# lliutianc/MPVAE-1

Measured on AMD Instinct MI355X. Metric: probit MC label-samples/sec (B×n_sample×L) at 1/2/4/8 GPU; ELBO rel-err, higher is better.
Workload: dtype f32; 1 GPU; c4: compute_loss fwd+bwd, B=512, L=1024, z=1024, n_sample=4096 (4096/GPU), philox noise on device; global_batch=512, n_sample=4096, label_dim=1024, z_dim=1024, parallelism=n_sample-sharded x1, gemm=f16x3

## Files before the change

mpvae-1_amd/csrc/mpv_common.h:

```cpp
#pragma once

#include <hip/hip_runtime.h>
#include <stdint.h>

#include "mpvae_hip.h"

#define MPV_DEV __device__ __forceinline__

namespace mpv {

constexpr float kEps1 = 1e-6f;
constexpr float kC1 = 1.0f - kEps1;
constexpr float kC0 = kEps1 * 0.5f;
constexpr float kInvSqrt2 = 0.70710678118654752440f;
constexpr float kInvSqrt2Pi = 0.39894228040143267794f;
constexpr float kKlEps = 1e-6f;
constexpr float kKlWeight = 1.1f;

typedef float f32x4 __attribute__((ext_vector_type(4)));

MPV_DEV float fast_log(float x) { return __builtin_amdgcn_logf(x) * 0.6931471805599453f; }
MPV_DEV float fast_rcp(float x) { return __builtin_amdgcn_rcpf(x); }

typedef float f32x2 __attribute__((ext_vector_type(2)));
// ... 238 lines not shown
      "v_fma_mixlo_f16 %1, %2, %3, -%0 op_sel_hi:[0,0,1]\n\t"
      "v_fma_mixhi_f16 %1, %2, %4, -%0 op_sel:[0,0,1] op_sel_hi:[0,0,1]"
      : "=&v"(h), "=&v"(l)
      : "s"(s), "v"(x0), "v"(x1), "v"(nz));
  hi = h;
  lo = l;
}

MPV_DEV float add_f32(float a, float b) {
  float r;
  asm("v_add_f32 %0, %1, %2" : "=v"(r) : "v"(a), "v"(b));
  return r;
}

MPV_DEV float pow2_scale(float maxabs) {
  if (!(maxabs > 0.0f) || !isfinite(maxabs)) return 1.0f;
  int e;
  frexpf(maxabs, &e);
  return ldexpf(1.0f, 14 - e);
}

MPV_DEV void bstat_combine_row(const float* __restrict__ g, int64_t R, int64_t B, int64_t b,
                               float (&v)[6]) {
#pragma unroll
  for (int br = 0; br < 2; ++br) {
    const int mi = 2 * br, zi = 2 * br + 1;
    float M = -INFINITY;
    for (int64_t r = 0; r < R; ++r) M = fmaxf(M, g[(r * 6 + mi) * B + b]);
    float Z = 0.0f;
    for (int64_t r = 0; r < R; ++r) Z += g[(r * 6 + zi) * B + b] * expf(g[(r * 6 + mi) * B + b] - M);
    v[mi] = M;
    v[zi] = Z;
  }
  for (int k = 4; k < 6; ++k) {
    float acc = 0.0f;
    for (int64_t r = 0; r < R; ++r) acc += g[(r * 6 + k) * B + b];
    v[k] = acc;
  }
}

MPV_DEV float wave_pow2_scale(const float* __restrict__ bound, int n) {
  float m = 0.0f;
  for (int i = threadIdx.x & 63; i < n; i += 64) m = fmaxf(m, bound[i]);
  return pow2_scale(wave_max(m));
}

MPV_DEV f16x8 as_f16x8(s16x8 v) { return __builtin_bit_cast(f16x8, v); }

constexpr int kLoOff = 32;
__host__ __device__ inline int64_t chunked_index(int64_t r, int64_t ld, int64_t c) {
  return r * ld + ((c >> 5) << 6) + (c & 31);
}

MPV_DEV void barrier_raw() {
  asm volatile("" ::: "memory");
  __builtin_amdgcn_s_barrier();
  asm volatile("" ::: "memory");
}

MPV_DEV void lds_barrier() {
  asm volatile("s_waitcnt lgkmcnt(0)" ::: "memory");
  barrier_raw();
}

template <int N>
MPV_DEV void wait_vmcnt() {
  asm volatile("s_waitcnt vmcnt(%0)" ::"n"(N) : "memory");
}

MPV_DEV uint32_t lds_addr(const void* p) {
  return (uint32_t)(uintptr_t)(const __attribute__((address_space(3))) void*)p;
}

MPV_DEV void lds_dma16(const void* saddr, uint32_t voff, uint32_t lds) {
  uint32_t keep;
  asm volatile(
      "s_mov_b32 %0, m0\n\ts_mov_b32 m0, %3\n\ts_nop 0\n\t"
      "global_load_lds_dwordx4 %1, %2\n\ts_mov_b32 m0, %0"
      : "=&s"(keep)
      : "v"(voff), "s"(saddr), "s"(lds)
      : "memory");
}

__host__ __device__ inline int64_t t_cols(int64_t L) { return (L + 3) & ~int64_t(3); }

MPV_DEV void wait_vmcnt_dyn(int n) {
#define MPV_VMC(k) \
  case k:          \
    wait_vmcnt<k>(); \
    break;
  switch (n) {
    MPV_VMC(0) MPV_VMC(1) MPV_VMC(2) MPV_VMC(3) MPV_VMC(4) MPV_VMC(5) MPV_VMC(6) MPV_VMC(7)
    MPV_VMC(8) MPV_VMC(9) MPV_VMC(10) MPV_VMC(11) MPV_VMC(12) MPV_VMC(13) MPV_VMC(14)
    MPV_VMC(15) MPV_VMC(16) MPV_VMC(17) MPV_VMC(18) MPV_VMC(19) MPV_VMC(20) MPV_VMC(21)
    MPV_VMC(22) MPV_VMC(23) MPV_VMC(24)
    default:
      wait_vmcnt<0>();
      break;
  }
#undef MPV_VMC
}

struct u32x4 { uint32_t x, y, z, w; };

MPV_DEV u32x4 philox4x32_10(u32x4 c, uint32_t k0, uint32_t k1) {
#pragma unroll
  for (int r = 0; r < 10; ++r) {
    const uint64_t p0 = (uint64_t)0xD2511F53u * c.x, p1 = (uint64_t)0xCD9E8D57u * c.z;
    const uint32_t lo0 = (uint32_t)p0, hi0 = (uint32_t)(p0 >> 32);
    const uint32_t lo1 = (uint32_t)p1, hi1 = (uint32_t)(p1 >> 32);
    c = u32x4{(uint32_t)__builtin_amdgcn_bitop3_b32(hi1, c.y, k0, 0x96), lo1,
              (uint32_t)__builtin_amdgcn_bitop3_b32(hi0, c.w, k1, 0x96), lo0};
    k0 += 0x9E3779B9u;
    k1 += 0xBB67AE85u;
  }
  return c;
}

MPV_DEV void box_muller(uint32_t we, uint32_t wo, float& n0, float& n1) {
  const float u = ((float)(we >> 8) + 0.5f) * 5.9604644775390625e-8f;
  const float v = (float)(wo >> 8) * 5.9604644775390625e-8f;
  const float r = __builtin_amdgcn_sqrtf(-1.3862943611198906f * __builtin_amdgcn_logf(u));
  n0 = r * __builtin_amdgcn_cosf(v);
  n1 = r * __builtin_amdgcn_sinf(v);
}

inline int num_cus() {
  static const int n = [] {
    int dev = 0, v = 0;
    if (hipGetDevice(&dev) != hipSuccess ||
        hipDeviceGetAttribute(&v, hipDeviceAttributeMultiprocessorCount, dev) != hipSuccess ||
        v <= 0)
      v = 256;
    return v;
  }();
  return n;
}

}
```

mpvae-1_amd/csrc/probit_bwd.hip:

```cpp
#include "abi_util.h"
#include "mpv_common.h"


namespace mpv {

int launch_sum_slabs(const float* in, int64_t nslab, int64_t n, void* out, int out_dtype,
                     hipStream_t s);
int launch_sum_slabs_pair(const float* in0, int64_t nslab0, int64_t n0, void* out0,
                          int out0_dtype, const float* in1, int64_t nslab1, int64_t n1,
                          void* out1, int out1_dtype, hipStream_t s);

constexpr float kBoundDl = 4.5f, kBoundPos = 0.4f, kBoundNeg = 60.0f, kBoundInd = 0.4f;

constexpr int kCoefThreads = 512;

__global__ __launch_bounds__(kCoefThreads) void bwd_coef_kernel(
    const float* __restrict__ y, const float* __restrict__ rowstat, const float* __restrict__ bstat,
    const float* __restrict__ gscal, const float* __restrict__ gI, const float* __restrict__ gIL,
    float* __restrict__ coef, float* __restrict__ gbound, int S, int B, int L, float S_total,
    float nll_coeff, float c_coeff, int live, mpv_kl_bwd_args kl, int kl_blocks) {
  __shared__ float red[48];
  if ((int)blockIdx.x >= B) {
    kl_bwd_range(kl, (int64_t)(blockIdx.x - B) * blockDim.x + threadIdx.x,
                 (int64_t)kl_blocks * blockDim.x);
    return;
  }
  const int b = blockIdx.x, tid = threadIdx.x;
  float np = 0.f, nn = 0.f, gi = 0.f;
  for (int l = tid; l < L; l += blockDim.x) {
    const int64_t o = (int64_t)b * L + l;
    const float v = y[o];
    np += (v == 1.0f) ? 1.0f : 0.0f;
    nn += (v == 0.0f) ? 1.0f : 0.0f;
    gi = fmaxf(gi, (gI ? fabsf(gI[o]) : 0.0f) + (gIL ? fabsf(gIL[o]) : 0.0f));
  }
  {
    const int lane = tid & 63, wid = tid >> 6, nw = (blockDim.x + 63) >> 6;
    np = wave_sum(np);
    nn = wave_sum(nn);
    gi = wave_max(gi);
    __syncthreads();
    if (lane == 0) red[wid] = np, red[16 + wid] = nn, red[32 + wid] = gi;
    __syncthreads();
    np = nn = 0.0f;
    gi = -INFINITY;
    for (int i = 0; i < nw; ++i) {
      np += red[i];
      nn += red[16 + i];
      gi = fmaxf(gi, red[32 + i]);
    }
  }
  const float nrm = np * nn;
  auto gs = [&](int k) { return (live & MPV_LIVE(k)) ? gscal[k] : 0.0f; };
  const float gt = gs(MPV_G_TOTAL);
  const float gn[2] = {gs(MPV_G_NLL) + nll_coeff * gt, gs(MPV_G_NLL_X) + nll_coeff * gt};
  const float gc[2] = {gs(MPV_G_C) + c_coeff * gt, gs(MPV_G_C_X) + c_coeff * gt};
  const bool clive[2] = {(live & (MPV_LIVE(MPV_G_TOTAL) | MPV_LIVE(MPV_G_C))) != 0,
                         (live & (MPV_LIVE(MPV_G_TOTAL) | MPV_LIVE(MPV_G_C_X))) != 0};
  const float inv_B = 1.0f / (float)B;
  float bound = kBoundInd * gi / S_total;
  float bmaxb[2];
#pragma unroll
  for (int br = 0; br < 2; ++br) {
    const float M = bstat[(2 * br) * B + b], Z = bstat[(2 * br + 1) * B + b];
    const bool dead = !(nrm > 0.0f) && clive[br];
    const float cs = gc[br] / (nrm * S_total * (float)B);
    float bmax = 0.0f;
    auto one = [&](float lp, float P, float N, float& ca, float& cp, float& cn) {
      float alpha = -gn[br] * (expf(lp - M) / Z) * inv_B;
      float bP = nrm > 0.0f ? cs * N : 0.0f;
      float bN = nrm > 0.0f ? cs * P : 0.0f;
      bmax = fmaxf(bmax, kBoundDl * fabsf(alpha) + kBoundPos * fabsf(bP) + kBoundNeg * fabsf(bN));
      if (dead) alpha = bP = bN = __builtin_nanf("");
      ca = alpha * kPhiK;
      cp = bP * kPhiK;
      cn = bN * kPhiK;
    };
    const float* rl = rowstat + ((int64_t)br * B + b) * S;
    const float* rp = rowstat + ((int64_t)(2 + 2 * br) * B + b) * S;
    const float* rn = rowstat + ((int64_t)(3 + 2 * br) * B + b) * S;
    float* ca = coef + ((int64_t)(3 * br + 0) * B + b) * S;
    float* cp = coef + ((int64_t)(3 * br + 1) * B + b) * S;
    float* cn = coef + ((int64_t)(3 * br + 2) * B + b) * S;
    if ((S & 3) == 0) {
      for (int s = 4 * tid; s < S; s += 4 * (int)blockDim.x) {
        const f32x4 lp = *reinterpret_cast<const f32x4*>(rl + s);
        const f32x4 P = *reinterpret_cast<const f32x4*>(rp + s);
        const f32x4 N = *reinterpret_cast<const f32x4*>(rn + s);
        float a[4], p[4], n[4];
#pragma unroll
        for (int j = 0; j < 4; ++j) one(lp[j], P[j], N[j], a[j], p[j], n[j]);
        *reinterpret_cast<f32x4*>(ca + s) = f32x4{a[0], a[1], a[2], a[3]};
        *reinterpret_cast<f32x4*>(cp + s) = f32x4{p[0], p[1], p[2], p[3]};
        *reinterpret_cast<f32x4*>(cn + s) = f32x4{n[0], n[1], n[2], n[3]};
      }
    } else {
      for (int s = tid; s < S; s += blockDim.x) one(rl[s], rp[s], rn[s], ca[s], cp[s], cn[s]);
    }
    bmaxb[br] = bmax;
  }
  block_reduce2<true>(bmaxb[0], bmaxb[1], red);
  bound += bmaxb[0];
  bound += bmaxb[1];
  if (tid == 0 && gbound) gbound[b] = bound;
}

struct ElemParams {
  const float* y;
  const float* fe;
  const float* fx;
  const float* gI;
  const float* gIL;
  const float* coef;
  float* T;
  uint16_t* g;
  const float* g_bound;
  int64_t gld;
  float* colpart;
  int S, B, L, Lc;
  int ldT;
  int TPR, RPI, rows_per_chunk;
  float inv_S;
};

struct ElemCol {
  f32x2 base[4];
  f32x2 gind[4];
  float y[4];
  bool soft[4];
  float qm[4];
  float sga[4];
  float wp[4], wn[4];
  bool pos[4];
  float kp, kn;
};

template <bool SOFT = true, bool NANCHK = true, bool SOFT_RCP = false>
MPV_DEV void d_elem2x4(const float (&t)[4], const ElemCol& c, f32x2 alpha, f32x2 rkp, f32x2 rkn,
                       f32x2 (&out)[4], const f32x2* rkq = nullptr, const f32x2* qc1 = nullptr) {
  f32x2 zq[4], w[4], ez[4];
#pragma unroll
  for (int q = 0; q < 4; ++q) zq[q] = pk_fma(splat2(t[q]), splat2(kZq), c.base[q]);
  probit_dw2xN_zq<4>(zq, w, ez, qc1);
#pragma unroll
  for (int q = 0; q < 4; ++q) {
    f32x2 E;
    {
#pragma clang fp contract(off)
      E = w[q] * kEh + splat2(kC0);
    }
    const f32x2 d = E + splat2(c.qm[q]);
    const f32x2 r = f32x2{fast_rcp(d.x), fast_rcp(d.y)};
    f32x2 dE;
    if (SOFT && c.soft[q]) {
      const f32x2 omE = splat2(1.0f) - E;
      const f32x2 dl = SOFT_RCP ? splat2(c.y[q]) * f32x2{fast_rcp(E.x), fast_rcp(E.y)} -
                                      splat2(1.0f - c.y[q]) * f32x2{fast_rcp(omE.x), fast_rcp(omE.y)}
                                : splat2(c.y[q]) / E - splat2(1.0f - c.y[q]) / omE;
      dE = pk_fma(alpha, dl, c.gind[q]);
    } else {
      dE = pk_fma(alpha, r, c.gind[q]);
    }
    const f32x2 rk = rkq   ? rkq[q]
                     : SOFT ? pk_fma(splat2(c.wn[q]), rkn, splat2(c.wp[q]) * rkp)
                            : (c.pos[q] ? rkp : rkn);
    const f32x2 a = w[q] * c.sga[q];
    dE = pk_fma(rk, f32x2{__builtin_amdgcn_exp2f(a.x), __builtin_amdgcn_exp2f(a.y)}, dE);
    out[q] = dE * ez[q];
  }
  if (NANCHK && (rkp.x != rkp.x || rkp.y != rkp.y)) {
#pragma unroll
    for (int q = 0; q < 4; ++q) {
      if (rkp.x != rkp.x) out[q].x = rkp.x;
      if (rkp.y != rkp.y) out[q].y = rkp.y;
    }
  }
}

MPV_DEV void elem_rank_coefs(const ElemCol& c, f32x2 bP, f32x2 bN, f32x2& rkp, f32x2& rkn) {
  rkp = splat2(c.kp) * -bP;
  rkn = splat2(c.kn) * bN;
}

struct ElemRow {
  f32x2 alpha, bP, bN;
  float t[4];
};

MPV_DEV void elem_row_load(ElemRow& r, const ElemParams& p, int b, int s, int c0,
                           const bool (&ok)[4]) {
  const int64_t cb = (int64_t)b * p.S + s;
  const int64_t BS = (int64_t)p.B * p.S;
  r.alpha = f32x2{p.coef[0 * BS + cb], p.coef[3 * BS + cb]};
  r.bP = f32x2{p.coef[1 * BS + cb], p.coef[4 * BS + cb]};
  r.bN = f32x2{p.coef[2 * BS + cb], p.coef[5 * BS + cb]};
  const float* row = p.T + cb * p.ldT;
  if (c0 < p.L) {
    const f32x4 v = __builtin_nontemporal_load(reinterpret_cast<const f32x4*>(row + c0));
    r.t[0] = v[0]; r.t[1] = v[1]; r.t[2] = v[2]; r.t[3] = v[3];
  } else {
#pragma unroll
    for (int q = 0; q < 4; ++q) r.t[q] = ok[q] ? row[c0 + q] : 0.0f;
  }
}

MPV_DEV void elem_col_setup(const ElemParams& p, int b, int c0, bool active, bool (&ok)[4],
                            ElemCol& ec) {
  const int L = p.L;
  ec.kp = exp2f((-5.0f * 1.4426950408889634f) * kC0);
  ec.kn = exp2f((5.0f * 1.4426950408889634f) * kC0);
#pragma unroll
  for (int q = 0; q < 4; ++q) {
    const int c = c0 + q;
    ok[q] = active && c < L;
    const int64_t o = (int64_t)b * L + (ok[q] ? c : 0);
    const float yv = ok[q] ? p.y[o] : 0.0f;
    const float fe = ok[q] ? p.fe[o] : 0.0f;
    const float fx = ok[q] ? p.fx[o] : 0.0f;
    const float gi = (ok[q] && p.gI) ? p.gI[o] * p.inv_S : 0.0f;
    const float gil = (ok[q] && p.gIL) ? p.gIL[o] * p.inv_S : 0.0f;
    ec.base[q] = f32x2{fe, fx} * kZq;
    ec.gind[q] = f32x2{gil, gi} * kPhiK;
    ec.y[q] = yv;
    ec.soft[q] = !(yv == 0.0f || yv == 1.0f);
    ec.qm[q] = yv == 0.0f ? -1.0f : 0.0f;
    const float sgx = (yv == 1.0f ? -5.0f : 5.0f) * 1.4426950408889634f;
    ec.sga[q] = sgx * kEh;
    ec.wp[q] = yv == 1.0f ? 1.0f : 0.0f;
    ec.wn[q] = yv == 0.0f ? 1.0f : 0.0f;
    ec.pos[q] = yv == 1.0f;
  }
}

constexpr int kElemLookahead = 1;
constexpr int kElemMinRows = 16;
template <bool PLANES>
__global__ __launch_bounds__(256, 3) void bwd_elem_kernel(ElemParams p) {
  constexpr int LA = kElemLookahead;
  __shared__ float cred[256 * 8];
  const int b = blockIdx.x, sc = blockIdx.y;
  const int tid = threadIdx.x;
  const int rsub = tid / p.TPR, cq = tid % p.TPR;
  const bool active = rsub < p.RPI;
  const int c0 = blockIdx.z * 1024 + cq * 4;
// ... 13 lines not shown
    for (int j = 0; j < LA; ++j)
      if (s0 + j * R < s_end) elem_row_load(buf[j], p, b, s0 + j * R, c0, ok);
    for (int s = s0; s < s_end; s += R) {
      if (s + LA * R < s_end) elem_row_load(buf[LA], p, b, s + LA * R, c0, ok);
      const ElemRow& cur = buf[0];
      const int64_t cb = (int64_t)b * S + s;
      float G[4];
      f32x2 g2[4];
      f32x2 rkp, rkn;
      elem_rank_coefs(ec, cur.bP, cur.bN, rkp, rkn);
      d_elem2x4(cur.t, ec, cur.alpha, rkp, rkn, g2);
#pragma unroll
      for (int q = 0; q < 4; ++q) {
        sg2[q] = sg2[q] + g2[q];
        G[q] = ok[q] ? g2[q].x + g2[q].y : 0.0f;
      }
      if (PLANES) {
        uint16_t h[4], l[4];
#pragma unroll
        for (int q = 0; q < 4; ++q) split_f16(G[q], gs, h[q], l[q]);
        const int64_t o = chunked_index(cb, p.gld, c0);
        const s16x4 hv{(short)h[0], (short)h[1], (short)h[2], (short)h[3]};
        const s16x4 lv{(short)l[0], (short)l[1], (short)l[2], (short)l[3]};
        __builtin_nontemporal_store(hv, reinterpret_cast<s16x4*>(p.g + o));
        __builtin_nontemporal_store(lv, reinterpret_cast<s16x4*>(p.g + o + kLoOff));
      } else {
        float* row = p.T + cb * p.ldT;
        if (c0 < L) {
          *reinterpret_cast<f32x4*>(row + c0) = f32x4{G[0], G[1], G[2], G[3]};
        } else {
#pragma unroll
          for (int q = 0; q < 4; ++q)
            if (ok[q]) row[c0 + q] = G[q];
        }
      }
#pragma unroll
      for (int j = 0; j < LA; ++j) buf[j] = buf[j + 1];
    }
  }
#pragma unroll
  for (int q = 0; q < 4; ++q) {
    cred[tid * 8 + q] = sg2[q].x;
    cred[tid * 8 + 4 + q] = sg2[q].y;
  }
  __syncthreads();
  for (int j = tid; j < p.TPR * 4; j += blockDim.x) {
    const int cqq = j >> 2, q = j & 3;
    const int c = blockIdx.z * 1024 + j;
    if (c < L) {
      float e = 0.f, x = 0.f;
      for (int r = 0; r < p.RPI; ++r) {
        e += cred[(r * p.TPR + cqq) * 8 + q];
        x += cred[(r * p.TPR + cqq) * 8 + 4 + q];
      }
      p.colpart[(((int64_t)sc * 2 + 0) * B + b) * L + c] = e;
      p.colpart[(((int64_t)sc * 2 + 1) * B + b) * L + c] = x;
    }
  }
}

constexpr int kElemRing = 8;
constexpr int kElemRingRows = 256;
constexpr int kElemRingMinRows = 128;
template <bool SOFT, bool MASK, bool NANCHK>
MPV_DEV void elem_ring_rows(const ElemParams& p, const ElemCol& ec, const bool (&ok)[4], bool live,
                            int b, int sb, int nrows, int c0, float gs, uint32_t voff,
                            float* myring, const float (*cf)[8], f32x2 (&sg2)[4]) {
  constexpr int NR = kElemRing;
  const int lane = threadIdx.x & 63;
  const int64_t rowb = (int64_t)b * p.S + sb;
  const char* tbase = reinterpret_cast<const char*>(p.T + rowb * p.ldT);
  const int64_t rstride = (int64_t)p.ldT * 4;
  auto issue = [&](int r) {
    lds_dma16(tbase + r * rstride, voff, lds_addr(myring + (r % NR) * 256));
  };
  const int pro = min(NR, nrows);
  for (int r = 0; r < pro; ++r) issue(r);
  uint32_t rsel[4];
#pragma unroll
  for (int q = 0; q < 4; ++q) rsel[q] = ec.pos[q] ? 0u : 16u;
  const uint32_t loffb = live ? 2u * (uint32_t)(((c0 >> 5) << 6) + (c0 & 31)) : 0u;
  f32x2 qc1 = splat2(kErfcxC1);
  asm volatile("" : "+v"(qc1));
  auto row = [&](int r) {
    const f32x4 tv = *reinterpret_cast<const f32x4*>(myring + (r % NR) * 256 + lane * 4);
    const float t[4] = {tv[0], tv[1], tv[2], tv[3]};
    f32x2 g2[4];
    const char* crow =
        reinterpret_cast<const char*>(&cf[0][0]) + __builtin_amdgcn_readfirstlane(r * 32);
    const f32x2 rkp = *reinterpret_cast<const f32x2*>(crow);
    const f32x2 rkn = *reinterpret_cast<const f32x2*>(crow + 16);
    if (SOFT) {
      const f32x2 alpha = *reinterpret_cast<const f32x2*>(crow + 8);
      d_elem2x4<SOFT, false, true>(t, ec, alpha, rkp, rkn, g2);
    } else {
      f32x2 rkq[4];
#pragma unroll
      for (int q = 0; q < 4; ++q) rkq[q] = *reinterpret_cast<const f32x2*>(crow + rsel[q]);
      const f32x2 alpha = *reinterpret_cast<const f32x2*>(crow + rsel[0] + 8);
      d_elem2x4<SOFT, false, true>(t, ec, alpha, rkp, rkn, g2, rkq, &qc1);
    }
    if (NANCHK && __builtin_amdgcn_readfirstlane((rkp.x != rkp.x || rkp.y != rkp.y) ? 1 : 0)) {
#pragma unroll
      for (int q = 0; q < 4; ++q) {
        if (rkp.x != rkp.x) g2[q].x = rkp.x;
        if (rkp.y != rkp.y) g2[q].y = rkp.y;
      }
    }
    float G[4];
#pragma unroll
    for (int q = 0; q < 4; ++q) {
      sg2[q] = sg2[q] + g2[q];
      G[q] = add_f32(g2[q].x, g2[q].y);
      if (MASK && !ok[q]) G[q] = 0.0f;
    }
    uint32_t hv[2], lv[2];
    split2_f16(G[0], G[1], gs, hv[0], lv[0]);
    split2_f16(G[2], G[3], gs, hv[1], lv[1]);
    const uint64_t ga = reinterpret_cast<uint64_t>(p.g + (rowb + r) * p.gld);
    const uint64_t grow =
        ((uint64_t)(uint32_t)__builtin_amdgcn_readfirstlane((uint32_t)(ga >> 32)) << 32) |
        (uint64_t)(uint32_t)__builtin_amdgcn_readfirstlane((uint32_t)ga);
    if (!MASK || live) {
      asm volatile("global_store_dwordx2 %0, %1, %2 nt\n\t"
                   "global_store_dwordx2 %0, %3, %2 offset:%4 nt"
                   :
                   : "v"(loffb), "v"(u32x2{hv[0], hv[1]}), "s"(grow), "v"(u32x2{lv[0], lv[1]}),
                     "i"(2 * kLoOff));
    }
    if (r + NR < nrows) issue(r + NR);
  };
  int r = 0;
  if (!SOFT && !MASK && !NANCHK) {
    for (; r < min(NR - 1, nrows); ++r) {
      wait_vmcnt_dyn(min(NR - 1, nrows - 1 - r) + 2 * r);
      row(r);
    }
    for (; r <= nrows - NR; ++r) {
      wait_vmcnt<3 * (NR - 1)>();
      row(r);
    }
  }
  for (; r < nrows; ++r) {
    wait_vmcnt_dyn(min(NR - 1, nrows - 1 - r) + 2 * min(r, NR - 1));
    row(r);
  }
}

__global__ __launch_bounds__(256, 3) void bwd_elem_ring_kernel(ElemParams p) {
  constexpr int NR = kElemRing, CR = kElemRingRows;
  __shared__ __attribute__((aligned(16))) float ring[4][NR][256];
  __shared__ __attribute__((aligned(16))) float cf[CR][8];
  const int b = blockIdx.x, sc = blockIdx.y, tid = threadIdx.x;
  const int wid = __builtin_amdgcn_readfirstlane(tid >> 6);
  const int c0 = blockIdx.z * 1024 + tid * 4;
  const int S = p.S, B = p.B, L = p.L;
  const float gs = wave_pow2_scale(p.g_bound, B);
  bool ok[4];
  ElemCol ec;
  elem_col_setup(p, b, c0, true, ok, ec);
  bool my_soft = false;
#pragma unroll
  for (int q = 0; q < 4; ++q) my_soft |= ok[q] && ec.soft[q];
  const bool soft_any = __syncthreads_or(my_soft) != 0;
  const bool wave_live = (int)(blockIdx.z * 1024 + wid * 256) < p.Lc;
  const bool wave_full = (int)(blockIdx.z * 1024 + wid * 256 + 256) <= min(L, p.Lc);
  const bool live = c0 < p.Lc;
  const int s_begin = sc * p.rows_per_chunk;
  const int s_end = min(S, s_begin + p.rows_per_chunk);
  const int64_t BS = (int64_t)B * S;
  const uint32_t voff = (uint32_t)((c0 < L ? c0 : 0) * 4);
  f32x2 sg2[4] = {splat2(0.f), splat2(0.f), splat2(0.f), splat2(0.f)};
  for (int sb = s_begin; sb < s_end; sb += CR) {
    const int nrows = min(CR, s_end - sb);
    __syncthreads();
    bool nan_row = false;
    for (int r = tid; r < nrows; r += 256) {
      const int64_t o = (int64_t)b * S + sb + r;
      const f32x2 alpha{p.coef[o], p.coef[3 * BS + o]};
      const f32x2 bP{p.coef[BS + o], p.coef[4 * BS + o]};
      const f32x2 bN{p.coef[2 * BS + o], p.coef[5 * BS + o]};
      f32x2 rkp, rkn;
      elem_rank_coefs(ec, bP, bN, rkp, rkn);
      nan_row |= bP.x != bP.x || bP.y != bP.y;
      *reinterpret_cast<f32x4*>(&cf[r][0]) = f32x4{rkp.x, rkp.y, alpha.x, alpha.y};
      *reinterpret_cast<f32x4*>(&cf[r][4]) = f32x4{rkn.x, rkn.y, alpha.x, alpha.y};
    }
    const bool nan_any = __syncthreads_or(nan_row) != 0;
    if (!wave_live) continue;
    float* myring = &ring[wid][0][0];
    if (soft_any || !wave_full || nan_any) {
      if (soft_any)
        elem_ring_rows<true, true, true>(p, ec, ok, live, b, sb, nrows, c0, gs, voff, myring, cf, sg2);
      else
        elem_ring_rows<false, true, true>(p, ec, ok, live, b, sb, nrows, c0, gs, voff, myring, cf, sg2);
    } else {
      elem_ring_rows<false, false, false>(p, ec, ok, live, b, sb, nrows, c0, gs, voff, myring, cf,
                                          sg2);
    }
  }
  __syncthreads();
  float* cred = &ring[0][0][0];
#pragma unroll
  for (int q = 0; q < 4; ++q) {
    cred[tid * 8 + q] = sg2[q].x;
    cred[tid * 8 + 4 + q] = sg2[q].y;
  }
  __syncthreads();
  for (int j = tid; j < 1024; j += 256) {
    const int c = blockIdx.z * 1024 + j;
    if (c < L) {
      p.colpart[(((int64_t)sc * 2 + 0) * B + b) * L + c] = cred[(j >> 2) * 8 + (j & 3)];
      p.colpart[(((int64_t)sc * 2 + 1) * B + b) * L + c] = cred[(j >> 2) * 8 + 4 + (j & 3)];
// ... 76 lines not shown
  const int wm = wid / WN, wn = wid % WN;
  const int lr = lane & 15, lg = lane >> 4;
  const int rows = p.B * p.S;
  const int q_begin = kc * p.rows_per_chunk;
  const int q_end = min(p.rows_pad, q_begin + p.rows_per_chunk);
  int dma_off[PER_WAVE];
#pragma unroll
  for (int i = 0; i < PER_WAVE; ++i) {
    const int pc = wid * PER_WAVE + i;
    const int pr = pc % (PIECES / 2);
    const int lrow = lane / (64 / RPP), lpos = lane % (64 / RPP);
    const int r = pr * RPP + lrow;
    const int u_lds = lpos >> 1, half = lpos & 1;
    const int u_src = u_lds ^ (r & 7);
    dma_off[i] = 4 * (pc < PIECES / 2 ? l0 : z0) + u_src * 32 + half * 16;
  }
  const int tq = lr >> 2, tp = lr & 3;
  const int r0 = lg * 4 + tq, r1 = r0 + 16, sw = r0 & 7;

  f32x4 acc[TM][TN];
#pragma unroll
  for (int m = 0; m < TM; ++m)
#pragma unroll
    for (int n = 0; n < TN; ++n) acc[m][n] = f32x4{0.f, 0.f, 0.f, 0.f};

  const int nst = (q_end - q_begin + kDrKR - 1) / kDrKR;
  for (int j = 0; j < P && j < nst; ++j)
    dr_issue<PER_WAVE, PIECES, RPP>(p, smem + j * STAGE, q_begin + j * kDrKR, rows, wid, dma_off);
  for (int ci = 0; ci < nst; ++ci) {
    if (P == 1)
      wait_vmcnt<0>();
    else
      wait_vmcnt_dyn(min(P - 1, nst - 1 - ci) * PER_WAVE);
    asm volatile("s_waitcnt lgkmcnt(0)" ::: "memory");
    barrier_raw();
    if (ci + P < nst)
      dr_issue<PER_WAVE, PIECES, RPP>(p, smem + ((ci + P) % kDrStages) * STAGE,
                                 q_begin + (ci + P) * kDrKR, rows, wid, dma_off);
    const char* base = smem + (ci % kDrStages) * STAGE;
    s16x8 ah[TM], al[TM], bh[TN], bl[TN];
#pragma unroll
    for (int m = 0; m < TM; ++m) {
      const int t = wm * TM + m, uh = (t >> 1) * 4 + (t & 1);
      const int ch = ((uh ^ sw) << 5) + tp * 8, cl = (((uh + 2) ^ sw) << 5) + tp * 8;
      ah[m] = __builtin_shufflevector(tr_read(base, r0 * ROWB + ch),
                                      tr_read(base, r1 * ROWB + ch), 0, 1, 2, 3, 4, 5, 6, 7);
      al[m] = __builtin_shufflevector(tr_read(base, r0 * ROWB + cl),
                                      tr_read(base, r1 * ROWB + cl), 0, 1, 2, 3, 4, 5, 6, 7);
    }
#pragma unroll
    for (int n = 0; n < TN; ++n) {
      const int t = wn * TN + n, uh = (t >> 1) * 4 + (t & 1);
      const int ch = ((uh ^ sw) << 5) + tp * 8, cl = (((uh + 2) ^ sw) << 5) + tp * 8;
      bh[n] = __builtin_shufflevector(tr_read(base + IMG, r0 * ROWB + ch),
                                      tr_read(base + IMG, r1 * ROWB + ch), 0, 1, 2, 3, 4, 5, 6, 7);
      bl[n] = __builtin_shufflevector(tr_read(base + IMG, r0 * ROWB + cl),
                                      tr_read(base + IMG, r1 * ROWB + cl), 0, 1, 2, 3, 4, 5, 6, 7);
    }
#pragma unroll
    for (int m = 0; m < TM; ++m)
#pragma unroll
      for (int n = 0; n < TN; ++n) {
        acc[m][n] = __builtin_amdgcn_mfma_f32_16x16x32_f16(as_f16x8(ah[m]), as_f16x8(bh[n]),
                                                           acc[m][n], 0, 0, 0);
        acc[m][n] = __builtin_amdgcn_mfma_f32_16x16x32_f16(as_f16x8(ah[m]), as_f16x8(bl[n]),
                                                           acc[m][n], 0, 0, 0);
        acc[m][n] = __builtin_amdgcn_mfma_f32_16x16x32_f16(as_f16x8(al[m]), as_f16x8(bh[n]),
                                                           acc[m][n], 0, 0, 0);
      }
  }
  const float inv = 1.0f / (wave_pow2_scale(p.g_bound, p.B) * *p.eps16.scale);
#pragma unroll
  for (int m = 0; m < TM; ++m)
#pragma unroll
    for (int n = 0; n < TN; ++n)
#pragma unroll
      for (int i = 0; i < 4; ++i) {
        const int l = l0 + (wm * TM + m) * 16 + lg * 4 + i;
        const int zc = z0 + (wn * TN + n) * 16 + lr;
        if (l < p.L && zc < p.z) p.slab[((int64_t)kc * p.L + l) * p.z + zc] = acc[m][n][i] * inv;
      }
}

template <int TM, int TN>
struct DrFrag {
  s16x8 ah[TM], al[TM], bh[TN], bl[TN];
};

template <int TM, int TN, int ROWB, int IMG>
MPV_DEV void dr_read(DrFrag<TM, TN>& f, const char* base, int wm, int wn, int r0, int r1, int sw,
                     int tp) {
#pragma unroll
  for (int m = 0; m < TM; ++m) {
    const int t = wm * TM + m, uh = (t >> 1) * 4 + (t & 1);
    const int ch = ((uh ^ sw) << 5) + tp * 8, cl = (((uh + 2) ^ sw) << 5) + tp * 8;
    f.ah[m] = __builtin_shufflevector(tr_read(base, r0 * ROWB + ch), tr_read(base, r1 * ROWB + ch),
                                      0, 1, 2, 3, 4, 5, 6, 7);
    f.al[m] = __builtin_shufflevector(tr_read(base, r0 * ROWB + cl), tr_read(base, r1 * ROWB + cl),
                                      0, 1, 2, 3, 4, 5, 6, 7);
  }
#pragma unroll
  for (int n = 0; n < TN; ++n) {
    const int t = wn * TN + n, uh = (t >> 1) * 4 + (t & 1);
    const int ch = ((uh ^ sw) << 5) + tp * 8, cl = (((uh + 2) ^ sw) << 5) + tp * 8;
    f.bh[n] = __builtin_shufflevector(tr_read(base + IMG, r0 * ROWB + ch),
                                      tr_read(base + IMG, r1 * ROWB + ch), 0, 1, 2, 3, 4, 5, 6, 7);
    f.bl[n] = __builtin_shufflevector(tr_read(base + IMG, r0 * ROWB + cl),
                                      tr_read(base + IMG, r1 * ROWB + cl), 0, 1, 2, 3, 4, 5, 6, 7);
  }
}

template <int TM, int TN, int ROWB, int IMG, int PER_WAVE, class Dma>
MPV_DEV void dr_read_dma(DrFrag<TM, TN>& f, const char* base, int wm, int wn, int r0, int r1,
                         int sw, int tp, Dma& dma, char* dst, int rows, int lane_u, int lane_h) {
  constexpr int STEPS = TM + TN;
  int lu = lane_u;
  asm volatile("" : "+v"(lu));
  const char* sp = dma.src;
  int nvalid = PER_WAVE;
  if (!dma.is_g) {
    const int over = dma.q - (rows - 1);
    if (over > 0) sp -= over * dma.row_b;
    nvalid = max(1, min(PER_WAVE, rows - dma.q));
  }
#pragma unroll
  for (int k = 0; k < STEPS; ++k) {
    const bool is_a = k < TM;
    const int t = is_a ? wm * TM + k : wn * TN + (k - TM), uh = (t >> 1) * 4 + (t & 1);
    const int ch = ((uh ^ sw) << 5) + tp * 8, cl = (((uh + 2) ^ sw) << 5) + tp * 8;
    const char* img = is_a ? base : base + IMG;
    const s16x8 hi = __builtin_shufflevector(tr_read(img, r0 * ROWB + ch), tr_read(img, r1 * ROWB + ch),
                                             0, 1, 2, 3, 4, 5, 6, 7);
    const s16x8 lo = __builtin_shufflevector(tr_read(img, r0 * ROWB + cl), tr_read(img, r1 * ROWB + cl),
                                             0, 1, 2, 3, 4, 5, 6, 7);
    if (is_a) {
      f.ah[k] = hi;
      f.al[k] = lo;
    } else {
      f.bh[k - TM] = hi;
      f.bl[k - TM] = lo;
    }
    __builtin_amdgcn_sched_barrier(0);
#pragma unroll
    for (int i = k * PER_WAVE / STEPS; i < (k + 1) * PER_WAVE / STEPS; ++i) {
      lds_dma16(sp, (uint32_t)(((lu ^ (i & 7)) << 5) + lane_h), lds_addr(dst + (dma.pc0 + i) * 1024));
      sp += (i + 1 < nvalid) ? dma.row_b : 0;
    }
    __builtin_amdgcn_sched_barrier(0);
  }
  dma.end();
}

template <int TM, int TN>
MPV_DEV void dr_mfma(f32x4 (&acc)[TM][TN], const DrFrag<TM, TN>& f) {
#pragma unroll
  for (int m = 0; m < TM; ++m)
#pragma unroll
    for (int n = 0; n < TN; ++n) {
      acc[m][n] = __builtin_amdgcn_mfma_f32_16x16x32_f16(as_f16x8(f.ah[m]), as_f16x8(f.bh[n]),
                                                         acc[m][n], 0, 0, 0);
      acc[m][n] = __builtin_amdgcn_mfma_f32_16x16x32_f16(as_f16x8(f.ah[m]), as_f16x8(f.bl[n]),
                                                         acc[m][n], 0, 0, 0);
      acc[m][n] = __builtin_amdgcn_mfma_f32_16x16x32_f16(as_f16x8(f.al[m]), as_f16x8(f.bh[n]),
                                                         acc[m][n], 0, 0, 0);
    }
}

template <int COUNT, int PIECES>
MPV_DEV void drs_issue_range(const Dr16Params& p, char* dst, int q0, int rows, int pc0, int l0,
                             int z0, int lane_u, int lane_h) {
#pragma unroll
  for (int i = 0; i < COUNT; ++i) {
    const int pc = pc0 + i;
    const bool is_g = pc < PIECES / 2;
    const int r = is_g ? pc : pc - PIECES / 2;
    const int q = q0 + r;
    const char* src = is_g ? reinterpret_cast<const char*>(p.g + (int64_t)q * p.gld + 2 * l0)
                           : reinterpret_cast<const char*>(p.eps16.data +
                                                           (int64_t)min(q, rows - 1) * p.eps16.ld +
                                                           2 * z0);
    lds_dma16(src, (uint32_t)(((lane_u ^ (r & 7)) << 5) + lane_h), lds_addr(dst + pc * 1024));
  }
}

template <int PER_WAVE, int PIECES, int WN>
struct DrsDma {
  const char* src;
  int64_t row_b;
  int q;
  int pc0;
  bool is_g;
  MPV_DEV void init(const Dr16Params& p, int q_first, int wn, int l0, int z0) {
    static_assert(PIECES / 2 == (WN / 2) * PER_WAVE, "G rows on the first half of the waves");
    static_assert(PER_WAVE % 8 == 0, "the source swizzle (row & 7) restarts with every share");
    const int pc = wn * PER_WAVE;
    is_g = pc < PIECES / 2;
    pc0 = pc;
    q = q_first + (is_g ? pc : pc - PIECES / 2);
    row_b = is_g ? p.gld * 2 : p.eps16.ld * 2;
    src = is_g ? reinterpret_cast<const char*>(p.g + (int64_t)q * p.gld + 2 * l0)
               : reinterpret_cast<const char*>(p.eps16.data + (int64_t)q * p.eps16.ld + 2 * z0);
  }
  MPV_DEV void end() {
    src += kDrKR * row_b;
    q += kDrKR;
  }
};

template <int WM, int WN, int TM, int TN>
__global__ __launch_bounds__(WM* WN * 64, 1) void dR16s_kernel(Dr16Params p) {
  static_assert(WM == 2, "two wave groups");
  constexpr int BL = WM * TM * 16, BZ = WN * TN * 16;
  static_assert(BL == BZ, "square tile: one LDS row layout for both operands");
  constexpr int ROWB = BL * 4;
  constexpr int IMG = kDrKR * ROWB;
  constexpr int STAGE = 2 * IMG;
  constexpr int PIECES = STAGE / 1024;
  constexpr int RPP = 1024 / ROWB;
  constexpr int PER_WAVE = PIECES / WN;
  static_assert(PIECES % WN == 0, "DMA pieces must split over the waves");
  __shared__ __attribute__((aligned(1024))) char smem[2 * STAGE];

  int kc, tile;
  decode_kc_tile(blockIdx.x, p.nKc, p.nLt * p.nZt, kc, tile);
  const int l0 = (tile / p.nZt) * BL, z0 = (tile % p.nZt) * BZ;
  const int tid = threadIdx.x, lane = tid & 63;
  const int wid = __builtin_amdgcn_readfirstlane(tid >> 6);
  const int wm = wid / WN, wn = wid % WN;
  const int grp = wm;
  const int lr = lane & 15, lg = lane >> 4;
  const int rows = p.B * p.S;
  const int q_begin = kc * p.rows_per_chunk;
  const int q_end = min(p.rows_pad, q_begin + p.rows_per_chunk);
  static_assert(RPP == 1, "one 1-KB row per DMA piece");
  const int lane_u = lane >> 1, lane_h = (lane & 1) * 16;
  const int tq = lr >> 2, tp = lr & 3;
  const int r0 = lg * 4 + tq, r1 = r0 + 16, sw = r0 & 7;

  f32x4 acc[TM][TN];
#pragma unroll
  for (int m = 0; m < TM; ++m)
#pragma unroll
    for (int n = 0; n < TN; ++n) acc[m][n] = f32x4{0.f, 0.f, 0.f, 0.f};

  const int nst = (q_end - q_begin + kDrKR - 1) / kDrKR;
  if (grp == 0 && nst > 0) {
    drs_issue_range<PIECES / WN, PIECES>(p, smem, q_begin, rows, wn * (PIECES / WN), l0, z0, lane_u,
                                         lane_h);
    wait_vmcnt<0>();
  }
  DrFrag<TM, TN> f;
  DrsDma<PER_WAVE, PIECES, WN> dma;
  if (grp == 0) dma.init(p, q_begin + kDrKR, wn, l0, z0);
  barrier_raw();
  if (grp == 0) {
    int i = 0;
    for (; i + 1 < nst; ++i) {
      dr_read_dma<TM, TN, ROWB, IMG, PER_WAVE>(f, smem + (i & 1) * STAGE, wm, wn, r0, r1, sw, tp,
                                               dma, smem + (1 - (i & 1)) * STAGE, rows, lane_u,
                                               lane_h);
      lds_barrier();
      __builtin_amdgcn_s_setprio(1);
      dr_mfma<TM, TN>(acc, f);
      __builtin_amdgcn_s_setprio(0);
      wait_vmcnt<0>();
      barrier_raw();
    }
    for (; i < nst; ++i) {
      dr_read<TM, TN, ROWB, IMG>(f, smem + (i & 1) * STAGE, wm, wn, r0, r1, sw, tp);
      lds_barrier();
      __builtin_amdgcn_s_setprio(1);
      dr_mfma<TM, TN>(acc, f);
      __builtin_amdgcn_s_setprio(0);
      barrier_raw();
    }
    barrier_raw();
  } else {
    barrier_raw();
    for (int i = 0; i < nst; ++i) {
      dr_read<TM, TN, ROWB, IMG>(f, smem + (i & 1) * STAGE, wm, wn, r0, r1, sw, tp);
      lds_barrier();
      __builtin_amdgcn_s_setprio(1);
      dr_mfma<TM, TN>(acc, f);
      __builtin_amdgcn_s_setprio(0);
      barrier_raw();
    }
  }
  const float inv = 1.0f / (wave_pow2_scale(p.g_bound, p.B) * *p.eps16.scale);
#pragma unroll
  for (int m = 0; m < TM; ++m)
#pragma unroll
    for (int n = 0; n < TN; ++n)
#pragma unroll
      for (int i = 0; i < 4; ++i) {
        const int l = l0 + (wm * TM + m) * 16 + lg * 4 + i;
        const int zc = z0 + (wn * TN + n) * 16 + lr;
        if (l < p.L && zc < p.z) p.slab[((int64_t)kc * p.L + l) * p.z + zc] = acc[m][n][i] * inv;
      }
}

struct DrParams {
  const float* G;
  const float* eps;
  float* slab;
  int S, B, L, z;
  int ldG;
  int nLt, nZt, nKc, rows_per_chunk;
};

constexpr int kDrBK = 32;

template <int TM, int TN>
__global__ __launch_bounds__(256) void dR_gemm_kernel(DrParams p) {
  constexpr int WM = 2, WN = 2;
  constexpr int BM = WM * TM * 16;
  constexpr int BN = WN * TN * 16;
  constexpr int LDG = BM + 16, LDE = BN + 16;
  constexpr int G4 = kDrBK * BM / 4, E4 = kDrBK * BN / 4;
  constexpr int GV = (G4 + 255) / 256, EV = (E4 + 255) / 256;
  __shared__ __attribute__((aligned(16))) float smem[kDrBK * (LDG + LDE)];
  float* Gs = smem;
  float* Es = smem + kDrBK * LDG;

  const int nT = p.nLt * p.nZt;
  int kc, tile;
  {
    const int id = blockIdx.x, K = p.nKc;
    const int full = (K / 8) * 8 * nT;
    if (id < full) {
      const int q = id / (8 * nT), r = id % (8 * nT);
      tile = r / 8;
      kc = q * 8 + (r % 8);
    } else {
      const int r = id - full, Kr = K % 8;
      tile = r / Kr;
      kc = (K / 8) * 8 + (r % Kr);
    }
  }
  const int l0 = (tile / p.nZt) * BM, z0 = (tile % p.nZt) * BN;
  const int tid = threadIdx.x, lane = tid & 63, wid = tid >> 6;
  const int wm = wid / WN, wn = wid % WN;
  const int lr = lane & 15, lg = lane >> 4;
  const int S = p.S, B = p.B, L = p.L, z = p.z;
  const int rows = B * S;
  const int q_begin = kc * p.rows_per_chunk;
  const int q_end = min(rows, q_begin + p.rows_per_chunk);
  const bool gvec = true, evec = (z & 3) == 0;

  f32x4 acc[TM][TN];
#pragma unroll
  for (int m = 0; m < TM; ++m)
#pragma unroll
    for (int n = 0; n < TN; ++n) acc[m][n] = f32x4{0.f, 0.f, 0.f, 0.f};

  f32x4 rg[GV], re[EV];
  auto load = [&](int q0) {
#pragma unroll
    for (int v = 0; v < GV; ++v) {
      const int idx = tid + v * 256;
      f32x4 x = {0.f, 0.f, 0.f, 0.f};
      if (idx < G4) {
        const int r = idx / (BM / 4), c = l0 + (idx % (BM / 4)) * 4;
        const int q = q0 + r;
// ... 322 lines not shown
```

Baseline: 77.76 billion label-samples/s.

## Skip zero-alpha element math and precompute LDS addresses in backward GEMM

In the non-soft backward element path, each row's alpha is checked to see whether it is zero across the wave. Zero rows take a specialised body that skips the E/reciprocal computation. Separately, the double-buffered backward GEMM now precomputes swizzled LDS read addresses once and flips them between stages. It also uses compile-time DMA offsets through a new m0-add inline asm helper, and drops row clamping except on the last prefetch iteration. Together these cut per-iteration address arithmetic and scalar overhead, at the cost of more code paths and reliance on inline asm clobbering m0.

```diff
diff --git a/mpvae-1_amd/csrc/mpv_common.h b/mpvae-1_amd/csrc/mpv_common.h
--- a/mpvae-1_amd/csrc/mpv_common.h
+++ b/mpvae-1_amd/csrc/mpv_common.h
@@ -344,6 +344,17 @@
       : "memory");
 }
 
+#pragma clang diagnostic push
+#pragma clang diagnostic ignored "-Winline-asm"
+template <int OFF>
+MPV_DEV void lds_dma16_at(const void* saddr, uint32_t voff, uint32_t lds) {
+  asm volatile("s_add_u32 m0, %2, %3\n\ts_nop 0\n\tglobal_load_lds_dwordx4 %0, %1"
+               :
+               : "v"(voff), "s"(saddr), "s"(lds), "n"(OFF)
+               : "memory", "m0", "scc");
+}
+#pragma clang diagnostic pop
+
 __host__ __device__ inline int64_t t_cols(int64_t L) { return (L + 3) & ~int64_t(3); }
 
 MPV_DEV void wait_vmcnt_dyn(int n) {
diff --git a/mpvae-1_amd/csrc/probit_bwd.hip b/mpvae-1_amd/csrc/probit_bwd.hip
--- a/mpvae-1_amd/csrc/probit_bwd.hip
+++ b/mpvae-1_amd/csrc/probit_bwd.hip
@@ -1,3 +1,5 @@
+#include <type_traits>
+
 #include "abi_util.h"
 #include "mpv_common.h"
 
@@ -135,7 +137,7 @@
   float kp, kn;
 };
 
-template <bool SOFT = true, bool NANCHK = true, bool SOFT_RCP = false>
+template <bool SOFT = true, bool NANCHK = true, bool SOFT_RCP = false, bool AZERO = false>
 MPV_DEV void d_elem2x4(const float (&t)[4], const ElemCol& c, f32x2 alpha, f32x2 rkp, f32x2 rkn,
                        f32x2 (&out)[4], const f32x2* rkq = nullptr, const f32x2* qc1 = nullptr) {
   f32x2 zq[4], w[4], ez[4];
@@ -144,22 +146,26 @@
   probit_dw2xN_zq<4>(zq, w, ez, qc1);
 #pragma unroll
   for (int q = 0; q < 4; ++q) {
-    f32x2 E;
-    {
+    f32x2 dE;
+    if (AZERO) {
+      dE = c.gind[q];
+    } else {
+      f32x2 E;
+      {
 #pragma clang fp contract(off)
-      E = w[q] * kEh + splat2(kC0);
-    }
-    const f32x2 d = E + splat2(c.qm[q]);
-    const f32x2 r = f32x2{fast_rcp(d.x), fast_rcp(d.y)};
-    f32x2 dE;
-    if (SOFT && c.soft[q]) {
-      const f32x2 omE = splat2(1.0f) - E;
-      const f32x2 dl = SOFT_RCP ? splat2(c.y[q]) * f32x2{fast_rcp(E.x), fast_rcp(E.y)} -
-                                      splat2(1.0f - c.y[q]) * f32x2{fast_rcp(omE.x), fast_rcp(omE.y)}
-                                : splat2(c.y[q]) / E - splat2(1.0f - c.y[q]) / omE;
-      dE = pk_fma(alpha, dl, c.gind[q]);
-    } else {
-      dE = pk_fma(alpha, r, c.gind[q]);
+        E = w[q] * kEh + splat2(kC0);
+      }
+      const f32x2 d = E + splat2(c.qm[q]);
+      const f32x2 r = f32x2{fast_rcp(d.x), fast_rcp(d.y)};
+      if (SOFT && c.soft[q]) {
+        const f32x2 omE = splat2(1.0f) - E;
+        const f32x2 dl = SOFT_RCP ? splat2(c.y[q]) * f32x2{fast_rcp(E.x), fast_rcp(E.y)} -
+                                        splat2(1.0f - c.y[q]) * f32x2{fast_rcp(omE.x), fast_rcp(omE.y)}
+                                  : splat2(c.y[q]) / E - splat2(1.0f - c.y[q]) / omE;
+        dE = pk_fma(alpha, dl, c.gind[q]);
+      } else {
+        dE = pk_fma(alpha, r, c.gind[q]);
+      }
     }
     const f32x2 rk = rkq   ? rkq[q]
                      : SOFT ? pk_fma(splat2(c.wn[q]), rkn, splat2(c.wp[q]) * rkp)
@@ -339,7 +345,8 @@
   const uint32_t loffb = live ? 2u * (uint32_t)(((c0 >> 5) << 6) + (c0 & 31)) : 0u;
   f32x2 qc1 = splat2(kErfcxC1);
   asm volatile("" : "+v"(qc1));
-  auto row = [&](int r) {
+  auto body = [&](int r, auto az) {
+    constexpr bool AZ = decltype(az)::value;
     const f32x4 tv = *reinterpret_cast<const f32x4*>(myring + (r % NR) * 256 + lane * 4);
     const float t[4] = {tv[0], tv[1], tv[2], tv[3]};
     f32x2 g2[4];
@@ -354,8 +361,9 @@
       f32x2 rkq[4];
 #pragma unroll
       for (int q = 0; q < 4; ++q) rkq[q] = *reinterpret_cast<const f32x2*>(crow + rsel[q]);
-      const f32x2 alpha = *reinterpret_cast<const f32x2*>(crow + rsel[0] + 8);
-      d_elem2x4<SOFT, false, true>(t, ec, alpha, rkp, rkn, g2, rkq, &qc1);
+      const f32x2 alpha =
+          AZ ? splat2(0.0f) : *reinterpret_cast<const f32x2*>(crow + rsel[0] + 8);
+      d_elem2x4<SOFT, false, true, AZ>(t, ec, alpha, rkp, rkn, g2, rkq, &qc1);
     }
     if (NANCHK && __builtin_amdgcn_readfirstlane((rkp.x != rkp.x || rkp.y != rkp.y) ? 1 : 0)) {
 #pragma unroll
@@ -386,6 +394,29 @@
                      "i"(2 * kLoOff));
     }
     if (r + NR < nrows) issue(r + NR);
+  };
+  auto alpha_bits = [&](int r) {
+    const char* crow =
+        reinterpret_cast<const char*>(&cf[0][0]) + __builtin_amdgcn_readfirstlane(r * 32);
+    const u32x2 a = *reinterpret_cast<const u32x2*>(crow + 8);
+    return a;
+  };
+  auto all_zero = [](u32x2 a) {
+    return ((uint32_t)__builtin_amdgcn_readfirstlane((int)(a[0] | a[1])) << 1) == 0u;
+  };
+  bool az_next = !SOFT && nrows > 0 && all_zero(alpha_bits(0));
+  auto row = [&](int r) {
+    if (SOFT) {
+      body(r, std::false_type{});
+      return;
+    }
+    const bool az = az_next;
+    const u32x2 an = alpha_bits(min(r + 1, nrows - 1));
+    if (az)
+      body(r, std::true_type{});
+    else
+      body(r, std::false_type{});
+    az_next = all_zero(an);
   };
   int r = 0;
   if (!SOFT && !MASK && !NANCHK) {
@@ -628,72 +659,109 @@
       }
 }
 
+template <int BEGIN, int END, class F>
+MPV_DEV void static_for(F&& f) {
+  if constexpr (BEGIN < END) {
+    f(std::integral_constant<int, BEGIN>{});
+    static_for<BEGIN + 1, END>(f);
+  }
+}
+
 template <int TM, int TN>
 struct DrFrag {
   s16x8 ah[TM], al[TM], bh[TN], bl[TN];
 };
 
 template <int TM, int TN, int ROWB, int IMG>
-MPV_DEV void dr_read(DrFrag<TM, TN>& f, const char* base, int wm, int wn, int r0, int r1, int sw,
-                     int tp) {
-#pragma unroll
-  for (int m = 0; m < TM; ++m) {
-    const int t = wm * TM + m, uh = (t >> 1) * 4 + (t & 1);
-    const int ch = ((uh ^ sw) << 5) + tp * 8, cl = (((uh + 2) ^ sw) << 5) + tp * 8;
-    f.ah[m] = __builtin_shufflevector(tr_read(base, r0 * ROWB + ch), tr_read(base, r1 * ROWB + ch),
-                                      0, 1, 2, 3, 4, 5, 6, 7);
-    f.al[m] = __builtin_shufflevector(tr_read(base, r0 * ROWB + cl), tr_read(base, r1 * ROWB + cl),
-                                      0, 1, 2, 3, 4, 5, 6, 7);
-  }
-#pragma unroll
-  for (int n = 0; n < TN; ++n) {
-    const int t = wn * TN + n, uh = (t >> 1) * 4 + (t & 1);
-    const int ch = ((uh ^ sw) << 5) + tp * 8, cl = (((uh + 2) ^ sw) << 5) + tp * 8;
-    f.bh[n] = __builtin_shufflevector(tr_read(base + IMG, r0 * ROWB + ch),
-                                      tr_read(base + IMG, r1 * ROWB + ch), 0, 1, 2, 3, 4, 5, 6, 7);
-    f.bl[n] = __builtin_shufflevector(tr_read(base + IMG, r0 * ROWB + cl),
-                                      tr_read(base + IMG, r1 * ROWB + cl), 0, 1, 2, 3, 4, 5, 6, 7);
-  }
-}
-
-template <int TM, int TN, int ROWB, int IMG, int PER_WAVE, class Dma>
-MPV_DEV void dr_read_dma(DrFrag<TM, TN>& f, const char* base, int wm, int wn, int r0, int r1,
-                         int sw, int tp, Dma& dma, char* dst, int rows, int lane_u, int lane_h) {
+struct DrAddr {
+  static_assert(TM % 4 == 0 && TN % 4 == 0, "a wave's tiles start at a multiple of four");
+  static_assert(IMG + 16 * ROWB + 256 * ((2 * TM - 1) / 4) < 65536, "ds offset field");
+  uint32_t a[8];
+  uint32_t bz;
+  MPV_DEV void init(uint32_t stage0, int r0, int tp, int wn) {
+#pragma unroll
+    for (int k = 0; k < 8; ++k) a[k] = stage0 + r0 * ROWB + ((k ^ (r0 & 7)) << 5) + tp * 8;
+    bz = 256u * (uint32_t)(wn * (TN / 4));
+  }
+  MPV_DEV void flip(int d) {
+#pragma unroll
+    for (int k = 0; k < 8; ++k) {
+      a[k] += d;
+      asm volatile("" : "+v"(a[k]));
+    }
+  }
+};
+
+MPV_DEV s16x4 tr_read_at(uint32_t addr, int off) {
+  return __builtin_amdgcn_ds_read_tr16_b64_v4i16(
+      (__attribute__((address_space(3))) s16x4*)(uintptr_t)(addr + off));
+}
+
+template <int TM, int TN, int ROWB, int IMG, int WMG>
+MPV_DEV void dr_read_tile(DrFrag<TM, TN>& f, const DrAddr<TM, TN, ROWB, IMG>& ad,
+                          const uint32_t (&b)[8], int j) {
+  const bool is_a = j < TM;
+  const int t = is_a ? WMG * TM + j : j - TM;
+  const int uh = (t >> 1) * 4 + (t & 1), kh = uh & 7, kl = kh + 2;
+  const int off = 256 * (uh >> 3) + (is_a ? 0 : IMG);
+  const uint32_t ah = is_a ? ad.a[kh] : b[kh], al = is_a ? ad.a[kl] : b[kl];
+  const s16x8 hi = __builtin_shufflevector(tr_read_at(ah, off), tr_read_at(ah, off + 16 * ROWB),
+                                           0, 1, 2, 3, 4, 5, 6, 7);
+  const s16x8 lo = __builtin_shufflevector(tr_read_at(al, off), tr_read_at(al, off + 16 * ROWB),
+                                           0, 1, 2, 3, 4, 5, 6, 7);
+  if (is_a) {
+    f.ah[j] = hi;
+    f.al[j] = lo;
+  } else {
+    f.bh[j - TM] = hi;
+    f.bl[j - TM] = lo;
+  }
+}
+
+template <int TM, int TN, int ROWB, int IMG, int WMG>
+MPV_DEV void dr_read(DrFrag<TM, TN>& f, const DrAddr<TM, TN, ROWB, IMG>& ad) {
+  uint32_t b[8];
+#pragma unroll
+  for (int k = 0; k < 8; ++k) b[k] = ad.a[k] + ad.bz;
+#pragma unroll
+  for (int j = 0; j < TM + TN; ++j) dr_read_tile<TM, TN, ROWB, IMG, WMG>(f, ad, b, j);
+}
+
+template <int TM, int TN, int ROWB, int IMG, int PER_WAVE, bool CLAMP, class Dma>
+MPV_DEV void dr_read_dma(DrFrag<TM, TN>& f, const DrAddr<TM, TN, ROWB, IMG>& ad, Dma& dma,
+                         uint32_t dst, int rows, int lane_v) {
   constexpr int STEPS = TM + TN;
-  int lu = lane_u;
-  asm volatile("" : "+v"(lu));
+  int lv = lane_v;
+  asm volatile("" : "+v"(lv));
   const char* sp = dma.src;
   int nvalid = PER_WAVE;
-  if (!dma.is_g) {
+  if (CLAMP && !dma.is_g) {
     const int over = dma.q - (rows - 1);
     if (over > 0) sp -= over * dma.row_b;
     nvalid = max(1, min(PER_WAVE, rows - dma.q));
   }
-#pragma unroll
-  for (int k = 0; k < STEPS; ++k) {
-    const bool is_a = k < TM;
-    const int t = is_a ? wm * TM + k : wn * TN + (k - TM), uh = (t >> 1) * 4 + (t & 1);
-    const int ch = ((uh ^ sw) << 5) + tp * 8, cl = (((uh + 2) ^ sw) << 5) + tp * 8;
-    const char* img = is_a ? base : base + IMG;
-    const s16x8 hi = __builtin_shufflevector(tr_read(img, r0 * ROWB + ch), tr_read(img, r1 * ROWB + ch),
-                                             0, 1, 2, 3, 4, 5, 6, 7);
-    const s16x8 lo = __builtin_shufflevector(tr_read(img, r0 * ROWB + cl), tr_read(img, r1 * ROWB + cl),
-                                             0, 1, 2, 3, 4, 5, 6, 7);
-    if (is_a) {
-      f.ah[k] = hi;
-      f.al[k] = lo;
-    } else {
-      f.bh[k - TM] = hi;
-      f.bl[k - TM] = lo;
-    }
+  const uint32_t dstw = dst + dma.pc0 * 1024;
+  uint32_t b[8];
+#pragma unroll
+  for (int k = 0; k < 8; ++k) b[k] = ad.a[k] + ad.bz;
+  static_for<0, STEPS>([&](auto kc) __attribute__((always_inline)) {
+    constexpr int k = decltype(kc)::value;
+    dr_read_tile<TM, TN, ROWB, IMG, 0>(f, ad, b, k);
     __builtin_amdgcn_sched_barrier(0);
-#pragma unroll
-    for (int i = k * PER_WAVE / STEPS; i < (k + 1) * PER_WAVE / STEPS; ++i) {
-      lds_dma16(sp, (uint32_t)(((lu ^ (i & 7)) << 5) + lane_h), lds_addr(dst + (dma.pc0 + i) * 1024));
-      sp += (i + 1 < nvalid) ? dma.row_b : 0;
-    }
+    static_for<k * PER_WAVE / STEPS, (k + 1) * PER_WAVE / STEPS>(
+        [&](auto ic) __attribute__((always_inline)) {
+          constexpr int i = decltype(ic)::value;
+          const uint32_t voff = (uint32_t)lv ^ ((i & 7) << 5);
+          if (CLAMP) {
+            lds_dma16(sp, voff, dstw + i * 1024);
+            sp += (i + 1 < nvalid) ? dma.row_b : 0;
+          } else {
+            lds_dma16_at<i * 1024>(sp, voff, dstw);
+            sp += dma.row_b;
+          }
+        });
     __builtin_amdgcn_sched_barrier(0);
-  }
+  });
   dma.end();
 }
 
@@ -780,8 +848,9 @@
   const int q_end = min(p.rows_pad, q_begin + p.rows_per_chunk);
   static_assert(RPP == 1, "one 1-KB row per DMA piece");
   const int lane_u = lane >> 1, lane_h = (lane & 1) * 16;
+  const int lane_v = (lane_u << 5) + lane_h;
   const int tq = lr >> 2, tp = lr & 3;
-  const int r0 = lg * 4 + tq, r1 = r0 + 16, sw = r0 & 7;
+  const int r0 = lg * 4 + tq;
 
   f32x4 acc[TM][TN];
 #pragma unroll
@@ -798,13 +867,18 @@
   DrFrag<TM, TN> f;
   DrsDma<PER_WAVE, PIECES, WN> dma;
   if (grp == 0) dma.init(p, q_begin + kDrKR, wn, l0, z0);
+  const uint32_t smem0 = lds_addr(smem);
+  DrAddr<TM, TN, ROWB, IMG> ad;
+  ad.init(smem0, r0, tp, wn);
   barrier_raw();
   if (grp == 0) {
     int i = 0;
-    for (; i + 1 < nst; ++i) {
-      dr_read_dma<TM, TN, ROWB, IMG, PER_WAVE>(f, smem + (i & 1) * STAGE, wm, wn, r0, r1, sw, tp,
-                                               dma, smem + (1 - (i & 1)) * STAGE, rows, lane_u,
-                                               lane_h);
+    int d = STAGE;
+    for (; i + 2 < nst; ++i) {
+      dr_read_dma<TM, TN, ROWB, IMG, PER_WAVE, false>(f, ad, dma, smem0 + (1 - (i & 1)) * STAGE,
+                                                      rows, lane_v);
+      ad.flip(d);
+      d = -d;
       lds_barrier();
       __builtin_amdgcn_s_setprio(1);
       dr_mfma<TM, TN>(acc, f);
@@ -812,8 +886,20 @@
       wait_vmcnt<0>();
       barrier_raw();
     }
+    for (; i + 1 < nst; ++i) {
+      dr_read_dma<TM, TN, ROWB, IMG, PER_WAVE, true>(f, ad, dma, smem0 + (1 - (i & 1)) * STAGE,
+                                                     rows, lane_v);
+      ad.flip(d);
+      d = -d;
+      lds_barrier();
+      __builtin_amdgcn_s_setprio(1);
+      dr_mfma<TM, TN>(acc, f);
+      __builtin_amdgcn_s_setprio(0);
+      wait_vmcnt<0>();
+      barrier_raw();
+    }
     for (; i < nst; ++i) {
-      dr_read<TM, TN, ROWB, IMG>(f, smem + (i & 1) * STAGE, wm, wn, r0, r1, sw, tp);
+      dr_read<TM, TN, ROWB, IMG, 0>(f, ad);
       lds_barrier();
       __builtin_amdgcn_s_setprio(1);
       dr_mfma<TM, TN>(acc, f);
@@ -823,8 +909,11 @@
     barrier_raw();
   } else {
     barrier_raw();
+    int d = STAGE;
     for (int i = 0; i < nst; ++i) {
-      dr_read<TM, TN, ROWB, IMG>(f, smem + (i & 1) * STAGE, wm, wn, r0, r1, sw, tp);
+      dr_read<TM, TN, ROWB, IMG, 1>(f, ad);
+      ad.flip(d);
+      d = -d;
       lds_barrier();
       __builtin_amdgcn_s_setprio(1);
       dr_mfma<TM, TN>(acc, f);
```

After: 78.48 billion label-samples/s (median of 6 runs). Within noise of the previous version (+0.9%).
